# South-Twilight/ParallelWaveGAN

Hardware: AMD Instinct MI355X
Metric: audio samples/sec/GPU (24 kHz PWG, 80-band mel) + RTF at 1/2/4/8 MI355X (higher is better)
Workload: dtype f32 (fp16 hi+lo pair operands, 3 f16 MFMAs per product, fp32 accumulate); 1 GPU; libritts_v1 generator inference, 32 ragged utterances per GPU per step; model=ParallelWaveGANGenerator, hop=300, global_batch=32, frames_per_gpu=24295, parallelism=1 process, 1 GPU (no collective)

## Files before the change

### include/pwg.h

```cpp
#ifndef PWG_H_
#define PWG_H_

#include <stddef.h>

#ifdef __cplusplus
extern "C" {
#endif

#define PWG_ABI_VERSION 2
#if defined(__GNUC__) || defined(__clang__)
#define PWG_API __attribute__((visibility("default")))
#else
#define PWG_API
#endif
#define PWG_MAX_SCALES 8

enum {
  PWG_OK = 0,
  PWG_ERR_INVALID = 1,
  PWG_ERR_ASSERT = 2,
  PWG_ERR_HIP = 3,
  PWG_ERR_UNSUPPORTED = 4,
  PWG_ERR_RANGE = 5,
  PWG_ERR_RERUN = 6
// ... 54 lines not shown
PWG_API long long pwg_plan_workspace_bytes(const PwgPlan* p);

PWG_API int pwg_run(PwgPlan* p, const float* packed, const float* mel, const float* noise,
            const float* mean, const float* scale, float* out, void* workspace, void* stream);

PWG_API int pwg_run_status(PwgPlan* p, const void* workspace, void* stream);

typedef struct PwgGraph PwgGraph;
PWG_API int pwg_graph_create(PwgPlan* p, const float* packed, const float* mel, const float* noise,
                             const float* mean, const float* scale, float* out, void* workspace, void* stream,
                             PwgGraph** out_graph);
PWG_API int pwg_graph_launch(PwgGraph* g, void* stream);
PWG_API void pwg_graph_destroy(PwgGraph* g);

enum {
  PWG_OPT_LAYER_KERNEL = 0,
  PWG_OPT_WAVES_PER_WG = 1,
  PWG_OPT_WG_PER_CU = 2,
  PWG_OPT_FUSE_FIRST_CONV = 3,
  PWG_OPT_PIPELINE = 4,
  PWG_OPT_HALF_BLOCKS = 5,
  PWG_OPT_SYNC = 6,
  PWG_OPT_SYNC_ABORT = 7,
  PWG_OPT_SYNC_TIMEOUT = 8
};
#define PWG_PIPE_MAX_DEFAULT 0LL
PWG_API int pwg_set_option(PwgHandle* h, int option, long long value);
PWG_API int pwg_get_option(const PwgHandle* h, int option, long long* value);

PWG_API int pwg_release_stream(PwgHandle* h, void* stream);
PWG_API int pwg_set_timing(PwgHandle* h, int enable);
PWG_API int pwg_timing_collect(PwgHandle* h, double* ms, long long* launches);
PWG_API int pwg_timing_span(PwgHandle* h, double* span_ms);

#define PWG_RCCL_UNIQUE_ID_BYTES 128
PWG_API int pwg_rccl_unique_id(void* id_out );
PWG_API int pwg_rccl_comm_create(int nranks, const void* id, int rank, int device, void** comm_out);
PWG_API int pwg_rccl_comm_destroy(void* comm);
PWG_API int pwg_broadcast_weights(const PwgHandle* h, void* comm, int root, float* packed, void* stream);

#ifdef __cplusplus
}
#endif
#endif
```

### parallelwavegan_amd/_lib.py

```python

import ctypes
import os
import subprocess
import threading

PKG_DIR = os.path.dirname(os.path.abspath(__file__))
REPO_DIR = os.path.dirname(PKG_DIR)
LIB_DIR = os.path.join(PKG_DIR, "lib")
LIB_PATH = os.environ.get("PWG_LIB_PATH") or os.path.join(LIB_DIR, "libpwg_hip.so")
CSRC = [
    os.path.join(PKG_DIR, "csrc", "pwg_kernels.hip"),
    os.path.join(PKG_DIR, "csrc", "pwg_capi.hip"),
    os.path.join(PKG_DIR, "csrc", "pwg_cnet.hip"),
    os.path.join(PKG_DIR, "csrc", "pwg_split.hip"),
    os.path.join(PKG_DIR, "csrc", "pwg_split16.hip"),
    os.path.join(PKG_DIR, "csrc", "pwg_rccl.hip"),
    os.path.join(PKG_DIR, "csrc", "pwg_mstack.hip"),
    os.path.join(PKG_DIR, "csrc", "pwg_rstack.hip"),
    os.path.join(PKG_DIR, "csrc", "pwg_embed.hip"),
]
HEADERS = [
    os.path.join(REPO_DIR, "include", "pwg.h"),
    os.path.join(REPO_DIR, "include", "pwg_cnet.h"),
    os.path.join(REPO_DIR, "include", "pwg_embed.h"),
# ... 18 lines not shown

EXPORTED_SYMBOLS = (
    "pwg_abi_version",
    "pwg_last_error",
    "pwg_create",
    "pwg_destroy",
    "pwg_receptive_field_size",
    "pwg_upsample_factor",
    "pwg_ref_weight_count",
    "pwg_packed_weight_count",
    "pwg_pack_weights",
    "pwg_plan_create",
    "pwg_plan_destroy",
    "pwg_plan_total_samples",
    "pwg_plan_padded_samples",
    "pwg_plan_workspace_bytes",
    "pwg_run",
    "pwg_run_status",
    "pwg_graph_create",
    "pwg_graph_launch",
    "pwg_graph_destroy",
    "pwg_set_option",
    "pwg_get_option",
    "pwg_set_timing",
    "pwg_release_stream",
    "pwg_timing_collect",
    "pwg_timing_span",
    "pwg_rccl_unique_id",
    "pwg_rccl_comm_create",
    "pwg_rccl_comm_destroy",
    "pwg_broadcast_weights",
    "pwg_cnet_abi_version",
    "pwg_cnet_create",
    "pwg_cnet_destroy",
    "pwg_cnet_packed_weight_count",
    "pwg_cnet_pack_weights",
    "pwg_cnet_plan_create",
    "pwg_cnet_plan_destroy",
    "pwg_cnet_plan_image",
    "pwg_cnet_plan_rows",
    "pwg_cnet_plan_workspace_bytes",
    "pwg_cnet_run",
    "pwg_cnet_run_status",
    "pwg_cnet_plan_schedule",
    "pwg_cnet_set_option",
    "pwg_cnet_set_timing",
    "pwg_cnet_timing_collect",
    "pwg_cnet_timing_span",
    "pwg_cnet_release_stream",
    "pwg_rstack_debug_launches",
    "pwg_rstack_debug_probe",
    "pwg_embed_rows",
)

PWG_OPT_LAYER_KERNEL = 0
PWG_OPT_WAVES_PER_WG = 1
PWG_OPT_WG_PER_CU = 2
PWG_OPT_FUSE_FIRST_CONV = 3
PWG_OPT_PIPELINE = 4
PWG_OPT_HALF_BLOCKS = 5
PWG_OPT_SYNC = 6
PWG_OPT_SYNC_ABORT = 7
PWG_OPT_SYNC_TIMEOUT = 8


class PwgConfig(ctypes.Structure):
    _fields_ = [
        ("in_channels", ctypes.c_int),
        ("out_channels", ctypes.c_int),
        ("kernel_size", ctypes.c_int),
        ("layers", ctypes.c_int),
        ("stacks", ctypes.c_int),
        ("residual_channels", ctypes.c_int),
        ("gate_channels", ctypes.c_int),
        ("skip_channels", ctypes.c_int),
        ("aux_channels", ctypes.c_int),
        ("aux_context_window", ctypes.c_int),
        ("use_causal_conv", ctypes.c_int),
        ("use_conv_in", ctypes.c_int),
        ("num_scales", ctypes.c_int),
        ("upsample_scales", ctypes.c_int * PWG_MAX_SCALES),
        ("interpolate_mode", ctypes.c_int),
    ]


def _needs_build():
# ... 136 lines not shown
        lib.pwg_abi_version.restype = ctypes.c_int
        lib.pwg_last_error.restype = ctypes.c_char_p
        lib.pwg_create.argtypes = [ctypes.POINTER(PwgConfig), ctypes.c_int, ctypes.POINTER(vp)]
        lib.pwg_destroy.argtypes = [vp]
        lib.pwg_destroy.restype = None
        for name in ("pwg_receptive_field_size", "pwg_upsample_factor", "pwg_ref_weight_count",
                     "pwg_packed_weight_count"):
            getattr(lib, name).argtypes = [vp]
            getattr(lib, name).restype = ll
        lib.pwg_pack_weights.argtypes = [vp, vp, vp]
        lib.pwg_plan_create.argtypes = [vp, ctypes.c_int, ctypes.POINTER(ll), ctypes.c_int, ctypes.POINTER(vp)]
        lib.pwg_plan_destroy.argtypes = [vp]
        lib.pwg_plan_destroy.restype = None
        for name in ("pwg_plan_total_samples", "pwg_plan_padded_samples", "pwg_plan_workspace_bytes"):
            getattr(lib, name).argtypes = [vp]
            getattr(lib, name).restype = ll
        lib.pwg_run.argtypes = [vp, vp, vp, vp, vp, vp, vp, vp, vp]
        lib.pwg_run_status.argtypes = [vp, vp, vp]
        lib.pwg_graph_create.argtypes = [vp] * 9 + [ctypes.POINTER(vp)]
        lib.pwg_graph_launch.argtypes = [vp, vp]
        lib.pwg_graph_destroy.argtypes = [vp]
        lib.pwg_graph_destroy.restype = None
        lib.pwg_get_option.argtypes = [vp, ctypes.c_int, ctypes.POINTER(ll)]
        lib.pwg_rccl_unique_id.argtypes = [vp]
        lib.pwg_rccl_comm_create.argtypes = [ctypes.c_int, vp, ctypes.c_int, ctypes.c_int, ctypes.POINTER(vp)]
        lib.pwg_rccl_comm_destroy.argtypes = [vp]
        lib.pwg_broadcast_weights.argtypes = [vp, vp, ctypes.c_int, vp, vp]
        lib.pwg_set_timing.argtypes = [vp, ctypes.c_int]
        lib.pwg_release_stream.argtypes = [vp, vp]
        lib.pwg_set_option.argtypes = [vp, ctypes.c_int, ctypes.c_longlong]
        lib.pwg_timing_collect.argtypes = [vp, ctypes.POINTER(ctypes.c_double), ctypes.POINTER(ll)]
        lib.pwg_timing_span.argtypes = [vp, ctypes.POINTER(ctypes.c_double)]
        lib.pwg_embed_rows.argtypes = [vp, ctypes.c_int, vp, ctypes.c_int, ctypes.c_int, vp, vp, vp, ctypes.c_int, ll,
                                       vp, vp, vp]
        if lib.pwg_abi_version() != 2:
            raise RuntimeError("libpwg_hip ABI version mismatch")
        _lib = lib
        return lib


class RangeError(ArithmeticError):
    """PWG_ERR_RANGE: a value left the fp16 pair range of the split-f16 kernels."""


class RerunError(RuntimeError):
    """PWG_ERR_RERUN: a grid-synchronised or layer-pipelined forward did not complete (the GPU was
# ... 20 lines not shown
```

### parallelwavegan_amd/csrc/pwg_capi.hip

```cpp
#include <hip/hip_runtime.h>

#include <algorithm>
#include <cmath>
#include <cstdio>
#include <cstdlib>
#include <cstring>
#include <map>
#include <mutex>
#include <string>
#include <utility>
#include <vector>

#include "../../include/pwg.h"
#include "pwg_internal.h"

#ifndef PWG_SMALL_SPREAD
#define PWG_SMALL_SPREAD 1
#endif

using namespace pwg;

namespace {

thread_local std::string g_err;
// ... 295 lines not shown

struct PwgHandle {
  PwgConfig cfg;
  int device;
  int R, RS, G, GH, GHPAD, GR, MT, S, SS, M2T, A, KS, KW, O, L, lps, K1, NQ, NQ4;
  long long gap;
  std::vector<int> dil;
  AuxStruct aux;
  size_t off_first_w, off_first_b, off_conv_in, off_conv_in_frag, off_waux;
  size_t off_tab_interior, off_tab_left, off_tab_right, off_tab_small;
  size_t off_layers, layer_stride, lo_wg, lo_bg, lo_w2;
  size_t off_head_w1, off_head_w2, off_head_b2, packed_total;
  int M3T;
  long long ref_total;
  size_t lo_wgp;
  int split_ok = 0;
  size_t lo_split = 0, off_skip0 = 0;
  size_t lo_split16 = 0, off_skip0_16 = 0, off_head16_w1 = 0, off_head16_w2 = 0;
  int layer_kernel = 0, waves_per_wg = 8, wg_per_cu = 1;
  int fuse_first = 1;
  long long pipe_max = PWG_PIPE_MAX_DEFAULT;
  int sync_abort = 0;
  int sync_timeout = 0;
  long long sync_max = -1;
  long long half_max = -1;
  int n_cu = 0;
  int* d_status = nullptr;
  std::string trace_fn;
  unsigned long long* d_trace = nullptr;
  size_t trace_words = 0;
  int timing = 0;
  std::vector<TimingRecord> records;
  std::vector<hipEvent_t> event_pool;
  std::map<hipStream_t, int*> hstatus;
  std::mutex hstatus_mu;
};

struct PwgPlan {
  PwgHandle* h;
  int layout;
  int n_utts;
  std::vector<UttDesc> utts;
  long long n_tiles, n_gap_tiles, Tpad, F_total, T_total;
  size_t ws_x0, ws_x1, ws_skip, ws_c1, ws_d, ws_ctr, ws_flag;
  size_t ws_utts, ws_tile_utt, ws_gap, ws_blocks, ws_total;
  bool pipe_ok = false;
// ... 550 lines not shown
    if (b) h->event_pool.push_back(b);
  };
  if (!a || !b || hipEventRecord(a, s) != hipSuccess) {
    give_back();
    return fail(PWG_ERR_HIP, "timing event");
  }
  const int rc = pwg_run_impl(p, packed, mel, noise, mean, scale, out, workspace, stream);
  if (hipEventRecord(b, s) != hipSuccess) {
    give_back();
    return fail(PWG_ERR_HIP, "timing event");
  }
  h->records.push_back({-1, a, b});
  return rc;
}

static int pwg_run_impl(PwgPlan* p, const float* packed, const float* mel, const float* noise, const float* mean,
                        const float* scale, float* out, void* workspace, void* stream) {
  if (!p || !packed || !mel || !noise || !out || !workspace) return fail(PWG_ERR_INVALID, "null argument");
  if (((uintptr_t)workspace & 255) != 0) return fail(PWG_ERR_INVALID, "workspace must be 256-byte aligned");
  if ((mean == nullptr) != (scale == nullptr)) return fail(PWG_ERR_INVALID, "mean and scale go together");
  if (mean != nullptr && p->layout != PWG_LAYOUT_INFERENCE)
    return fail(PWG_ERR_INVALID, "normalize_before is an inference() option");
  PwgHandle* h = p->h;
  DeviceGuard g(h->device);
  if (!g.ok) return fail(PWG_ERR_HIP, "hipSetDevice failed");
  if (h->n_cu == 0) {
    int n = 0;
    if (hipDeviceGetAttribute(&n, hipDeviceAttributeMultiprocessorCount, h->device) != hipSuccess || n < 1)
      return fail(PWG_ERR_HIP, "cannot query the CU count");
    h->n_cu = n;
  }
  if (h->d_status == nullptr) {
    if (hipMalloc((void**)&h->d_status, 256) != hipSuccess) return fail(PWG_ERR_HIP, "status word allocation");
    if (hipMemset(h->d_status, 0, 256) != hipSuccess) return fail(PWG_ERR_HIP, "status word reset");
  }
  hipStream_t s = (hipStream_t)stream;
  char* ws = (char*)workspace;
  float* x0 = (float*)(ws + p->ws_x0);
  float* x1 = (float*)(ws + p->ws_x1);
  float* skip = (float*)(ws + p->ws_skip);
  float* c1 = (float*)(ws + p->ws_c1);
  float* dproj = (float*)(ws + p->ws_d);
  int* sched_ctr = (int*)(ws + p->ws_ctr);

  auto timed = [&](int bucket, auto&& launch) -> hipError_t {
    if (h->timing != 1) return launch();
// ... 241 lines not shown
      if (fuse_first && l == 0) {
        sa.noise = noise; sa.fw = packed + h->off_first_w; sa.fb = packed + h->off_first_b;
      }
      const int launch_w = split16 ? std::min(8, h->waves_per_wg) : wpw;
      if (split16 && units > 8LL * h->n_cu && units <= 32LL * h->n_cu) wpw = std::min(wpw, 4);
      sa.compute_waves = std::min(wpw, launch_w);
      const bool trace_on = split16 && !h->trace_fn.empty();
      const size_t per_layer_s = (size_t)nwg * launch_w * 8;
      if (trace_on) {
        const size_t need = per_layer_s * 64;
        if (need > h->trace_words) {
          if (h->d_trace) {
            (void)hipStreamSynchronize(s);
            (void)hipFree(h->d_trace);
            h->d_trace = nullptr;
            h->trace_words = 0;
          }
          if (hipMalloc((void**)&h->d_trace, need * sizeof(unsigned long long)) != hipSuccess)
            return fail(PWG_ERR_HIP, "trace buffer");
          h->trace_words = need;
        }
        sa.trace = h->d_trace + per_layer_s * (l % 64);
      }
      e = timed(PWG_KERNEL_RESIDUAL_LAYER, [&] {
        return split16 ? launch_layer_split16(sa, last, la.tap_center, launch_w, nwg, s, half)
                       : launch_layer_split(sa, last, la.tap_center, wpw, nwg, s);
      });
      if (e == hipSuccess && last && trace_on) {
        std::vector<unsigned long long> host(per_layer_s * std::min(h->L, 64));
        e = hipStreamSynchronize(s);
        if (e == hipSuccess) e = hipMemcpy(host.data(), h->d_trace, host.size() * 8, hipMemcpyDeviceToHost);
        FILE* f = e == hipSuccess ? fopen(h->trace_fn.c_str(), "wb") : nullptr;
        if (f) {
          const long long hdr[4] = {std::min(h->L, 64), nwg, launch_w, 8};
          fwrite(hdr, sizeof(hdr), 1, f);
          fwrite(host.data(), 8, host.size(), f);
          fclose(f);
        }
      }
    } else if (h->layer_kernel == 0 && h->aux.nka <= 4) {
      PersistArgs pa2;
      pa2.x_in = xin; pa2.x_out = xout; pa2.skip = skip; pa2.d = la.d;
      pa2.tab = packed + h->off_tab_interior;
      pa2.tab_left = (int)(h->off_tab_left - h->off_tab_interior);
      pa2.tab_right = (int)(h->off_tab_right - h->off_tab_interior);
      pa2.tab_small = (int)(h->off_tab_small - h->off_tab_interior);
      pa2.blocks = d_blocks;
      pa2.wgp = la.wgp; pa2.w2 = la.w2; pa2.bg = la.bg;
// ... 149 lines not shown
      if (value < 1 || value > 64) return fail(PWG_ERR_INVALID, "workgroups per CU must be in [1, 64]");
      h->wg_per_cu = (int)value;
      return PWG_OK;
    case PWG_OPT_PIPELINE:
      if (value < 0) return fail(PWG_ERR_INVALID, "pipeline plan limit must be >= 0");
      h->pipe_max = value;
      return PWG_OK;
    case PWG_OPT_HALF_BLOCKS:
      if (value < 0) return fail(PWG_ERR_INVALID, "half-block limit must be >= 0");
      h->half_max = value;
      return PWG_OK;
    case PWG_OPT_SYNC:
      if (value < 0) return fail(PWG_ERR_INVALID, "grid-synchronised plan limit must be >= 0");
      h->sync_max = value;
      return PWG_OK;
    case PWG_OPT_SYNC_ABORT:
      if (value != 0 && value != 1) return fail(PWG_ERR_INVALID, "sync_abort must be 0 or 1");
      h->sync_abort = (int)value;
      return PWG_OK;
    case PWG_OPT_SYNC_TIMEOUT:
      if (value != 0 && value != 1) return fail(PWG_ERR_INVALID, "sync_timeout must be 0 or 1");
      h->sync_timeout = (int)value;
      return PWG_OK;

    default:
      return fail(PWG_ERR_INVALID, "unknown option");
  }
}

int pwg_get_option(const PwgHandle* h, int option, long long* value) {
  if (!h || !value) return fail(PWG_ERR_INVALID, "null argument");
  switch (option) {
    case PWG_OPT_LAYER_KERNEL: *value = h->layer_kernel; return PWG_OK;
    case PWG_OPT_WAVES_PER_WG: *value = h->waves_per_wg; return PWG_OK;
    case PWG_OPT_FUSE_FIRST_CONV: *value = h->fuse_first; return PWG_OK;
    case PWG_OPT_WG_PER_CU: *value = h->wg_per_cu; return PWG_OK;
    case PWG_OPT_PIPELINE: *value = h->pipe_max; return PWG_OK;
    case PWG_OPT_HALF_BLOCKS: *value = h->half_max >= 0 ? h->half_max : 4LL * h->n_cu; return PWG_OK;
    case PWG_OPT_SYNC: *value = h->sync_max >= 0 ? h->sync_max : 64LL * h->n_cu; return PWG_OK;
    case PWG_OPT_SYNC_ABORT: *value = h->sync_abort; return PWG_OK;
    case PWG_OPT_SYNC_TIMEOUT: *value = h->sync_timeout; return PWG_OK;

    default: return fail(PWG_ERR_INVALID, "unknown option");
  }
}

int pwg_release_stream(PwgHandle* h, void* stream) {
  if (!h) return fail(PWG_ERR_INVALID, "null handle");
  std::lock_guard<std::mutex> lk(h->hstatus_mu);
  auto it = h->hstatus.find((hipStream_t)stream);
  if (it == h->hstatus.end()) return PWG_OK;
  DeviceGuard g(h->device);
  if (stream && hipStreamSynchronize((hipStream_t)stream) != hipSuccess) return fail(PWG_ERR_HIP, "stream synchronize");
  (void)hipHostFree(it->second);
  h->hstatus.erase(it);
  return PWG_OK;
}

int pwg_set_timing(PwgHandle* h, int enable) {
  if (!h) return fail(PWG_ERR_INVALID, "null handle");
  if (enable < 0 || enable > 2) return fail(PWG_ERR_INVALID, "timing mode must be 0, 1 or 2");
  h->timing = enable;
  return PWG_OK;
}

int pwg_timing_collect(PwgHandle* h, double* ms, long long* launches) {
  if (!h || !ms || !launches) return fail(PWG_ERR_INVALID, "null argument");
// ... 60 lines not shown
```

### parallelwavegan_amd/csrc/pwg_internal.h

```cpp
#pragma once
#include <hip/hip_runtime.h>
#include <stdint.h>

namespace pwg {

constexpr int TILE = 128;
constexpr int KC = 16;
constexpr int MAX_SCALES = 8;
constexpr int AUX_J4 = 8;
constexpr int AUX_MAX_NFWG = 16;

struct UttDesc {
  long long seg_base;
  long long first_tile;
  long long T;
  long long frame_base;
  long long frames;
  long long mel_off;
  long long io_off;
};

struct ConvInArgs {
  const float* mel;
  const float* mean;
// ... 180 lines not shown
  UttDesc utts[PLAN_CHUNK];
  int n;
  int u0;
  int gap_tiles;
  int H;
  UttDesc* d_utts;
  int* tile_utt;
  long long* gap_col0;
  BlockDesc* blocks;
  int* zero;
  int n_zero;
  int* prog;
  unsigned* zx[3];
};
hipError_t launch_plan_desc(const PlanDescArgs& a, long long max_blocks, hipStream_t s);

hipError_t launch_conv_in(const ConvInArgs& a, hipStream_t s);
hipError_t launch_aux_proj(const AuxProjArgs& a, int layers, hipStream_t s);
hipError_t launch_first_conv(const FirstConvArgs& a, long long n_tiles, hipStream_t s);
hipError_t launch_layer(const LayerArgs& a, int mt, int m2t, bool last, long long n_tiles, hipStream_t s);
hipError_t launch_first_conv_split(const FirstConvArgs& a, long long n_tiles, hipStream_t s);
hipError_t launch_first_conv_split16(const FirstConvArgs& a, long long n_tiles, hipStream_t s);
hipError_t launch_layer_split16(const SplitArgs& a, bool last, int tap_center, int waves_per_wg, int n_wg,
                                hipStream_t s, bool half = false);
hipError_t launch_layer_split(const SplitArgs& a, bool last, int tap_center, int waves_per_wg, int n_wg,
                              hipStream_t s);
hipError_t launch_pipe_split16(const PipeArgs& p, int tap_center, int n_wg, hipStream_t s);
hipError_t launch_sync_split16(const SyncArgs& p, int tap_center, int n_wg, hipStream_t s);
hipError_t launch_layer_persistent(const PersistArgs& a, int mt, int m2t, bool last, int waves_per_wg, int n_wg,
                                   hipStream_t s);

template <typename V>
__device__ __forceinline__ void stage_lds(V* dst, const V* src, int n, int tid, int nthr) {
  int i = tid;
  for (; i + 7 * nthr < n; i += 8 * nthr) {
    V r[8];
#pragma unroll
    for (int j = 0; j < 8; ++j) r[j] = src[i + j * nthr];
#pragma unroll
    for (int j = 0; j < 8; ++j) dst[i + j * nthr] = r[j];
  }
  for (; i < n; i += nthr) dst[i] = src[i];
}

constexpr int MS_MAX = 4;
struct MsStack {
  const float* wA;
// ... 80 lines not shown
```

### parallelwavegan_amd/csrc/pwg_split16.hip

```cpp
#include "pwg_internal.h"


namespace pwg {

namespace {

typedef float f32x4 __attribute__((ext_vector_type(4)));
typedef _Float16 f16x8 __attribute__((ext_vector_type(8)));
typedef unsigned u32x4 __attribute__((ext_vector_type(4)));

__device__ __forceinline__ f32x4 mma16(u32x4 a, u32x4 b, f32x4 c) {
  return __builtin_amdgcn_mfma_f32_16x16x32_f16(__builtin_bit_cast(f16x8, a), __builtin_bit_cast(f16x8, b), c, 0, 0,
                                                0);
}

__device__ __forceinline__ float gate16(float u, float v) {
  u = fminf(u, 64.f);
  const float e1 = __builtin_amdgcn_exp2f(u);
  const float e2 = __builtin_amdgcn_exp2f(v);
  return (1.f - e1) * __builtin_amdgcn_rcpf((1.f + e1) * (1.f + e2));
}

template <int NOPS>
__device__ __forceinline__ void split8x(const float (&v)[8], u32x4& hi, u32x4& lo) {
// ... 24 lines not shown
  asm volatile(
      "v_fma_mix_f32 %0, %8, %16, %12 op_sel_hi:[1,0,0]\n\t"
      "v_fma_mix_f32 %1, %8, %16, %13 op_sel:[1,0,0] op_sel_hi:[1,0,0]\n\t"
      "v_fma_mix_f32 %2, %9, %16, %14 op_sel_hi:[1,0,0]\n\t"
      "v_fma_mix_f32 %3, %9, %16, %15 op_sel:[1,0,0] op_sel_hi:[1,0,0]\n\t"
      "v_fma_mix_f32 %4, %10, %16, %17 op_sel_hi:[1,0,0]\n\t"
      "v_fma_mix_f32 %5, %10, %16, %18 op_sel:[1,0,0] op_sel_hi:[1,0,0]\n\t"
      "v_fma_mix_f32 %6, %11, %16, %19 op_sel_hi:[1,0,0]\n\t"
      "v_fma_mix_f32 %7, %11, %16, %20 op_sel:[1,0,0] op_sel_hi:[1,0,0]\n\t"
      "v_fma_mix_f32 %0, %21, %16, %0 op_sel_hi:[1,0,0]\n\t"
      "v_fma_mix_f32 %1, %21, %16, %1 op_sel:[1,0,0] op_sel_hi:[1,0,0]\n\t"
      "v_fma_mix_f32 %2, %22, %16, %2 op_sel_hi:[1,0,0]\n\t"
      "v_fma_mix_f32 %3, %22, %16, %3 op_sel:[1,0,0] op_sel_hi:[1,0,0]\n\t"
      "v_fma_mix_f32 %4, %23, %16, %4 op_sel_hi:[1,0,0]\n\t"
      "v_fma_mix_f32 %5, %23, %16, %5 op_sel:[1,0,0] op_sel_hi:[1,0,0]\n\t"
      "v_fma_mix_f32 %6, %24, %16, %6 op_sel_hi:[1,0,0]\n\t"
      "v_fma_mix_f32 %7, %24, %16, %7 op_sel:[1,0,0] op_sel_hi:[1,0,0]\n\t"
      "s_nop 1"
      : "=&v"(o[0]), "=&v"(o[1]), "=&v"(o[2]), "=&v"(o[3]), "=&v"(o[4]), "=&v"(o[5]), "=&v"(o[6]), "=&v"(o[7])
      : "v"(l[0]), "v"(l[1]), "v"(l[2]), "v"(l[3]), "v"(b0[0]), "v"(b0[1]), "v"(b0[2]), "v"(b0[3]), "v"(c),
        "v"(b1[0]), "v"(b1[1]), "v"(b1[2]), "v"(b1[3]), "v"(h[0]), "v"(h[1]), "v"(h[2]), "v"(h[3]));
}

struct Pair16 {
  unsigned hi, lo;
};
__device__ __forceinline__ Pair16 split_pair16(float v0, float v1) {
  typedef _Float16 f16x2 __attribute__((ext_vector_type(2)));
  const _Float16 h0 = (_Float16)v0, h1 = (_Float16)v1;
  const _Float16 l0 = (_Float16)(v0 - (float)h0), l1 = (_Float16)(v1 - (float)h1);
  return {__builtin_bit_cast(unsigned, f16x2{h0, h1}), __builtin_bit_cast(unsigned, f16x2{l0, l1})};
}

}

__device__ __forceinline__ unsigned shifted16(int r, int g, int c) {
  const unsigned s = (unsigned)(r + c);
  return (unsigned)g * 256u + (s >> 4) * 4096u + (s & 15u) * 16u;
}

__device__ __forceinline__ BlockDesc uniform_desc(const BlockDesc& d) {
  BlockDesc u;
  u.col = __builtin_amdgcn_readfirstlane(d.col);
  u.t0 = __builtin_amdgcn_readfirstlane(d.t0);
  u.T = __builtin_amdgcn_readfirstlane(d.T);
  u.frames = __builtin_amdgcn_readfirstlane(d.frames);
// ... 114 lines not shown
#pragma unroll
    for (int m = 0; m < 4; ++m) {
      dv[j][m] = d0[m];
      dv[j][m + 4] = d1[m];
    }
  }
}

template <bool PIPE, int NTN = 2>
__device__ __forceinline__ void s16_load_skip(const SplitArgs& a, const BlockDesc& bd, f32x4 (&sk)[4][2], int g,
                                              int c, int h16 = 0) {
  const Plane16<PIPE> skip(a.skip);
  const long long sb = (long long)((bd.col + h16) >> 4) * 4096;
  const unsigned vo = 16u * (unsigned)(16 * g + c);
#pragma unroll
  for (int nt = 0; nt < NTN; ++nt)
#pragma unroll
    for (int ms = 0; ms < 4; ++ms) {
      if (a.first) sk[ms][nt] = reinterpret_cast<const f32x4*>(a.skip0 + 16 * g)[ms];
      else sk[ms][nt] = __builtin_bit_cast(f32x4, skip.template load<true>(sb + nt * 4096, vo, ms * 1024));
    }
}

template <bool LAST, int TC, bool FIRST, bool PIPE, int NTN = 2, bool AL = false, typename Mid>
__device__ __forceinline__ void s16_block(const SplitArgs& a, const unsigned* smem16, const BlockDesc& bd_v,
                                          const BlockDesc& bdn_v, bool has_next, u32x4 (&b0)[8], u32x4 (&b1)[8],
                                          bool& nonfinite, Mid&& mid, int h16_v = 0, int h16n_v = 0,
                                          bool poison = false) {
  static_assert(NTN == 2 || !LAST, "half blocks: middle layers");
  const BlockDesc bd = uniform_desc(bd_v);
  const int h16 = NTN == 1 ? __builtin_amdgcn_readfirstlane(h16_v) : 0;
  const unsigned* s_wg = smem16;
  const unsigned* s_w2 = s_wg + Split16Smem::WG;
  const unsigned* s_bg = s_w2 + Split16Smem::W2;
  const float* s_bo = reinterpret_cast<const float*>(s_bg + Split16Smem::BG);
  const float* s_hw1 = s_bo + Split16Smem::BO;
  const float* s_fwb = reinterpret_cast<const float*>(smem16 + Split16Smem::dwords(LAST));
  const int lane = threadIdx.x & 63;
  const int g = lane >> 4;
  const int c = lane & 15;
  constexpr int T1 = TC == 1 ? 2 : 1;
  const bool full = bd.t0 + h16 + 16 * NTN <= bd.T;

  unsigned dv[2][8];
  float bw[2][2];
  const bool two_frames = a.H >= 32;
  const int rem0 = bd.t0 - bd.f0 * a.H;
// ... 33 lines not shown
    for (int ks = 0; ks < 2; ++ks) {
#pragma unroll
      for (int mh = 0; mh < 2; ++mh) {
        u32x4 ah[4], al[4];
#pragma unroll
        for (int mm = 0; mm < 4; ++mm) {
          const int m = 4 * mh + mm;
          ah[mm] = wgl[(((tap * 2 + ks) * 8 + m) * 2) * 64];
          al[mm] = wgl[(((tap * 2 + ks) * 8 + m) * 2 + 1) * 64];
        }
#pragma unroll
        for (int mm = 0; mm < 4; ++mm)
#pragma unroll
          for (int nt = 0; nt < NTN; ++nt) {
            f32x4& ac = acc[4 * mh + mm][nt];
            ac = mma16(ah[mm], b[nt * 4 + ks * 2], ac);
            ac = mma16(ah[mm], b[nt * 4 + ks * 2 + 1], ac);
            ac = mma16(al[mm], b[nt * 4 + ks * 2], ac);
          }
        __builtin_amdgcn_sched_barrier(0);
      }
    }
  };

  f32x4 acc[8][2];
#pragma unroll
  for (int m = 0; m < 8; ++m)
#pragma unroll
    for (int nt = 0; nt < NTN; ++nt) acc[m][nt] = f32x4{0.f, 0.f, 0.f, 0.f};
  f32x4 acc2[8][2];
  s16_bload<TC, FIRST, PIPE, NTN, AL>(a, s_fwb, bd, T1, b1, g, c, h16);
  mma_tap(acc, b0, 0);
  s16_load_dv(a, bd, dv, g, c);
  s16_bload<TC, FIRST, PIPE, NTN, AL>(a, s_fwb, bd, TC, b0, g, c, h16);
  mma_tap(acc, b1, T1);
  mma_tap(acc, b0, TC);
  if (!LAST) {
    const f32x4* bo_l = reinterpret_cast<const f32x4*>(s_bo + 16 * g);
#pragma unroll
    for (int nt = 0; nt < NTN; ++nt)
#pragma unroll
      for (int ks = 0; ks < 2; ++ks) {
        float o[8];
        seed8x(b0[nt * 4 + ks * 2], b0[nt * 4 + ks * 2 + 1], bo_l[2 * ks], bo_l[2 * ks + 1], 0.70710677f, o);
#pragma unroll
        for (int j = 0; j < 8; ++j) acc2[4 + 2 * ks + (j >> 2)][nt][j & 3] = o[j];
      }
  }
  mid();

  {
    f32x4 sk[4][2];
    s16_load_skip<PIPE, NTN>(a, bd, sk, g, c, h16);
#pragma unroll
    for (int nt = 0; nt < NTN; ++nt)
#pragma unroll
      for (int ms = 0; ms < 4; ++ms) acc2[ms][nt] = sk[ms][nt];
  }

// ... 18 lines not shown
  }

  u32x4 gh[2][2], gl[2][2];
#pragma unroll
  for (int nt = 0; nt < NTN; ++nt)
#pragma unroll
    for (int ks = 0; ks < 2; ++ks) {
      float gv[8];
#pragma unroll
      for (int j = 0; j < 8; ++j) {
        const int m = 2 * ks + (j >> 2), i = j & 3;
        gv[j] = gate16(acc[m][nt][i], acc[m + 4][nt][i]);
      }
      split8x<0>(gv, gh[nt][ks], gl[nt][ks]);
    }

  if (has_next) {
    const BlockDesc bdn = uniform_desc(bdn_v);
    const int h16n = NTN == 1 ? __builtin_amdgcn_readfirstlane(h16n_v) : 0;
    s16_bload<TC, FIRST, PIPE, NTN, AL>(a, s_fwb, bdn, 0, b0, g, c, h16n);
  }
  constexpr int M2 = LAST ? 4 : 8;
  const u32x4* w2l = reinterpret_cast<const u32x4*>(s_w2) + lane;
#pragma unroll
  for (int ks = 0; ks < 2; ++ks)
#pragma unroll
    for (int mh = 0; mh < M2 / 4; ++mh) {
      u32x4 ah[4], al[4];
#pragma unroll
      for (int mm = 0; mm < 4; ++mm) {
        ah[mm] = w2l[((ks * 8 + 4 * mh + mm) * 2) * 64];
        al[mm] = w2l[((ks * 8 + 4 * mh + mm) * 2 + 1) * 64];
      }
#pragma unroll
      for (int mm = 0; mm < 4; ++mm)
#pragma unroll
        for (int nt = 0; nt < NTN; ++nt) {
          f32x4& ac = acc2[4 * mh + mm][nt];
          ac = mma16(ah[mm], gh[nt][ks], ac);
          ac = mma16(ah[mm], gl[nt][ks], ac);
          ac = mma16(al[mm], gh[nt][ks], ac);
        }
      __builtin_amdgcn_sched_barrier(0);
    }

  if (!LAST) {
    const Plane16<PIPE> skip(a.skip), xo(a.x_out);
    const long long sb = (long long)((bd.col + h16) >> 4) * 4096;
    const unsigned vo = 16u * (unsigned)lane;
#pragma unroll
    for (int nt = 0; nt < NTN; ++nt) {
      const bool live = bd.t0 + h16 + 16 * nt + c < bd.T;
#pragma unroll
      for (int ms = 0; ms < 4; ++ms)
        skip.store(sb + nt * 4096, vo, ms * 1024, __builtin_bit_cast(u32x4, acc2[ms][nt]));
#pragma unroll
      for (int ks = 0; ks < 2; ++ks) {
        float v[8];
#pragma unroll
        for (int j = 0; j < 8; ++j) v[j] = acc2[4 + 2 * ks + (j >> 2)][nt][j & 3];
        u32x4 vh, vl;
        split8x<11>(v, vh, vl);
        if (!full) {
#pragma unroll
          for (int k = 0; k < 4; ++k) {
            vh[k] = live ? vh[k] : 0u;
            vl[k] = live ? vl[k] : 0u;
// ... 49 lines not shown
      }
#pragma unroll
    for (int nt = 0; nt < 2; ++nt) {
      const int t = bd.t0 + 16 * nt + c;
      const bool live = t < bd.T;
      float* out = a.out + (size_t)bd.io_off * a.O + (size_t)t * a.out_stride_t;
      for (int oc = 0; oc < a.O; ++oc) {
        const f32x4* w = reinterpret_cast<const f32x4*>(a.hw2 + ((size_t)oc * 4 + g) * 16);
        float part = 0.f;
#pragma unroll
        for (int m3 = 0; m3 < 4; ++m3) {
          const f32x4 wq = w[m3];
#pragma unroll
          for (int i = 0; i < 4; ++i) part = fmaf(wq[i], fmaxf(acc3[m3][nt][i], 0.f), part);
        }
        part += __shfl_xor(part, 16);
        part += __shfl_xor(part, 32);
        if (g == 0 && live) out[(size_t)oc * a.out_stride_o] = poison ? __builtin_nanf("") : part + a.hb2[oc];
      }
    }
  }
}

template <bool LAST, int TC, bool FIRST, bool AL, int NTN>
__global__ void __launch_bounds__(512, 1) pwg_layer_split16_kernel(const SplitArgs a) {
  constexpr int UB = NTN == 1 ? 1 : 0;
  const int n_units = a.n_blocks << UB;
  extern __shared__ __attribute__((aligned(16))) unsigned smem16[];
  const bool tr = a.trace != nullptr;
  unsigned long long t_start = 0, c_start = 0, t_staged = 0, t_first = 0;
  if (tr) {
    t_start = __builtin_amdgcn_s_memrealtime();
    c_start = __builtin_amdgcn_s_memtime();
  }
  const int lane = threadIdx.x & 63;
  const int nw = a.compute_waves;
  const int xcd = blockIdx.x & 7;
  const int wave = threadIdx.x >> 6;
  const int blk0 = wave < nw ? (int)((long long)n_units * xcd / 8) + (blockIdx.x >> 3) * nw + wave : -1;
  bool poison = false;
  if constexpr (LAST)
    if (a.range_flag != nullptr)
      poison = (__hip_atomic_load(a.range_flag, __ATOMIC_RELAXED, __HIP_MEMORY_SCOPE_AGENT) & PWG_STATUS_REDO) != 0;
  const bool has0 = blk0 >= 0 && blk0 < (int)((long long)n_units * (xcd + 1) / 8);
  BlockDesc bdn;
  int h16n = 0;
  u32x4 b0[8], b1[8];
// ... 47 lines not shown
    return -1;
  };

  int blk = x_first + (blockIdx.x >> 3) * nw + wave;
  int nblk = blk + x_waves;
  if (blk >= x_end) blk = -1;
  if (nblk >= x_end) nblk = -1;
  if (blk < 0) {
    trace_out();
    return;
  }
  const float* s_fwb = reinterpret_cast<const float*>(smem16 + Split16Smem::dwords(LAST));
  if constexpr (FIRST)
    s16_bload<TC, true, false, NTN>(a, s_fwb, uniform_desc(bdn), 0, b0, lane >> 4, lane & 15,
                                    NTN == 1 ? __builtin_amdgcn_readfirstlane(h16n) : 0);
  bool nonfinite = false;
  while (true) {
    const BlockDesc bd = bdn;
    const int h16 = h16n;
    const int pf = nblk >= 0 ? nblk : blk;
    bdn = a.blocks[pf >> UB];
    h16n = NTN == 1 ? 16 * (pf & 1) : 0;
    int ticket = 0;
    s16_block<LAST, TC, FIRST, false, NTN, AL>(a, smem16, bd, bdn, true, b0, b1, nonfinite, [&]() {
      if (nblk >= 0) ticket = ticket_issue();
    }, h16, h16n, poison);
    if (tr && n_done++ == 0) t_first = __builtin_amdgcn_s_memrealtime();
    if (nblk < 0) break;
    blk = nblk;
    nblk = ticket_resolve(ticket);
  }
  if (LAST && nonfinite && a.range_flag) flag_status(a.range_flag, a.sticky, PWG_STATUS_RANGE);
  trace_out();
}

constexpr int PIPE_SPIN_LIMIT = 1 << 20;

template <bool LAST, int TC, bool FIRST>
__device__ __forceinline__ void pipe_layer(const PipeArgs& p, int l, unsigned* smem16) {
  SplitArgs a = p.base;
  a.wg = p.wg0 + (size_t)l * p.wg_stride;
  a.d = p.d0 + (size_t)l * p.d_stride;
  a.x_in = p.x[l % 3];
  a.x_out = p.x[(l + 1) % 3];
  a.dil = p.dil[l];
  a.first = l == 0;
  if (!FIRST) a.noise = nullptr;
// ... 203 lines not shown
    const long long t = t0 + jcol;
    unsigned v = 0u;
    if (t < ud.T) {
      const float z = a.noise[ud.io_off + t];
      float y[2];
#pragma unroll
      for (int e = 0; e < 2; ++e) {
        const int j = 2 * dw + e;
        const int ch = 16 * (2 * ks + (j >> 2)) + 4 * g + (j & 3);
        y[e] = fmaf(a.w[ch], z, a.b[ch]);
      }
      const Pair16 pr = split_pair16(y[0], y[1]);
      v = hl ? pr.lo : pr.hi;
    }
    x[(size_t)col0 * 64 + idx] = v;
  }
}

hipError_t launch_first_conv_split16(const FirstConvArgs& a, long long n_tiles, hipStream_t s) {
  hipLaunchKernelGGL(pwg_first_conv_split16_kernel, dim3((unsigned)n_tiles), dim3(256), 0, s, a);
  return hipGetLastError();
}

hipError_t launch_layer_split16(const SplitArgs& a, bool last, int tap_center, int waves_per_wg, int n_wg,
                                hipStream_t s, bool half) {
  if (waves_per_wg > 8) waves_per_wg = 8;
  if (a.compute_waves < 1 || a.compute_waves > waves_per_wg) return hipErrorInvalidValue;
  if (half && last) return hipErrorInvalidValue;
  const dim3 grid((unsigned)n_wg), block((unsigned)(64 * waves_per_wg));
#define PWG_SPLIT16_LAUNCH(LAST_, TC_, FIRST_, NTN_, AL_)                                               \
  {                                                                                                     \
    const size_t lds = sizeof(unsigned) * (Split16Smem::dwords(LAST_) + (FIRST_ ? 128 : 0));            \
    auto kfn = &pwg_layer_split16_kernel<LAST_, TC_, FIRST_, AL_, NTN_>;                                \
    hipError_t e_ = allow_lds(reinterpret_cast<const void*>(kfn), (int)lds);                           \
    if (e_ != hipSuccess) return e_;                                                                    \
    hipLaunchKernelGGL(kfn, grid, block, lds, s, a);                                                    \
    return hipGetLastError();                                                                           \
  }
  const bool first = a.noise != nullptr;
  if (first && last) return hipErrorInvalidValue;
  const bool al = a.dil % 16 == 0;
#define PWG_SPLIT16_MIDDLE(TC_, NTN_) \
  { if (al) PWG_SPLIT16_LAUNCH(false, TC_, false, NTN_, true) else PWG_SPLIT16_LAUNCH(false, TC_, false, NTN_, false) }
  if (tap_center == 1) {
    if (half) {
      if (first) PWG_SPLIT16_LAUNCH(false, 1, true, 1, false) else PWG_SPLIT16_MIDDLE(1, 1)
    }
    if (first) PWG_SPLIT16_LAUNCH(false, 1, true, 2, false)
    if (last) PWG_SPLIT16_LAUNCH(true, 1, false, 2, false) else PWG_SPLIT16_MIDDLE(1, 2)
  } else if (tap_center == 2) {
    if (half) {
      if (first) PWG_SPLIT16_LAUNCH(false, 2, true, 1, false) else PWG_SPLIT16_MIDDLE(2, 1)
    }
    if (first) PWG_SPLIT16_LAUNCH(false, 2, true, 2, false)
    if (last) PWG_SPLIT16_LAUNCH(true, 2, false, 2, false) else PWG_SPLIT16_MIDDLE(2, 2)
  }
#undef PWG_SPLIT16_MIDDLE
#undef PWG_SPLIT16_LAUNCH
  return hipErrorInvalidValue;
}

hipError_t launch_sync_split16(const SyncArgs& p, int tap_center, int n_wg, hipStream_t s) {
  const size_t lds = sizeof(unsigned) * (Split16Smem::dwords(false) + 128);
  if (p.L < 1 || p.L > PIPE_MAX_LAYERS || p.waves_mid < 1 || p.waves_mid > 8) return hipErrorInvalidValue;
  if (n_wg < 8) return hipErrorInvalidValue;
  auto kfn = tap_center == 1 ? (p.half ? &pwg_sync_split16_kernel<1, 1> : &pwg_sync_split16_kernel<1, 2>)
             : tap_center == 2 ? (p.half ? &pwg_sync_split16_kernel<2, 1> : &pwg_sync_split16_kernel<2, 2>)
                               : nullptr;
  if (kfn == nullptr) return hipErrorInvalidValue;
  const hipError_t e = allow_lds(reinterpret_cast<const void*>(kfn), (int)lds);
  if (e != hipSuccess) return e;
  hipLaunchKernelGGL(kfn, dim3((unsigned)n_wg), dim3(512), lds, s, p);
  return hipGetLastError();
}

hipError_t launch_pipe_split16(const PipeArgs& p, int tap_center, int n_wg, hipStream_t s) {
  const size_t lds = sizeof(unsigned) * (Split16Smem::dwords(true) > Split16Smem::dwords(false) + 128
                                             ? Split16Smem::dwords(true) : Split16Smem::dwords(false) + 128);
  if (n_wg < p.L || n_wg % 8 != 0) return hipErrorInvalidValue;
  auto kfn = tap_center == 1 ? &pwg_pipe_split16_kernel<1> : tap_center == 2 ? &pwg_pipe_split16_kernel<2> : nullptr;
  if (kfn == nullptr) return hipErrorInvalidValue;
// ... 8 lines not shown
```

### parallelwavegan_amd/engine.py

```python

import ctypes
import logging
import os
import operator
from collections import OrderedDict

import numpy as np
import torch

from . import _lib


def _scales(params):
    return list(params.get("upsample_params", {}).get("upsample_scales", [4, 4, 4, 4]))


def make_config(params):
    up = dict(params.get("upsample_params", {"upsample_scales": [4, 4, 4, 4]}))
    if not params.get("upsample_conditional_features", True):
        raise NotImplementedError("upsample_conditional_features=False is not supported")
    net = params.get("upsample_net", "ConvInUpsampleNetwork")
    if net not in ("ConvInUpsampleNetwork", "UpsampleNetwork"):
        raise NotImplementedError(f"upsample_net={net!r} is not supported")
    if up.get("nonlinear_activation") is not None:
# ... 310 lines not shown
    def release_stream(self, stream):
        key = stream.cuda_stream
        self._workspaces.pop(key, None)
        _lib.check(self._lib.pwg_release_stream(self._h, ctypes.c_void_p(key)))

    LAYER_KERNELS = {"persistent": 0, "tiled": 1, "split": 2, "split16": 3}

    def set_option(self, option, value):
        opts = self._OPTS
        if option == "layer_kernel" and isinstance(value, str):
            value = self.LAYER_KERNELS[value]
        if option == "layer_kernel" and int(value) in (2, 3) and not self.split_range_ok:
            raise _lib.RangeError("the loaded weights exceed the fp16 pair range of the split-f16 layer kernels")
        _lib.check(self._lib.pwg_set_option(self._h, opts[option], int(value)))
        if option == "layer_kernel":
            self.layer_kernel = int(value)
        if option == "pipeline":
            self._plans = OrderedDict()

    _OPTS = {"layer_kernel": _lib.PWG_OPT_LAYER_KERNEL, "waves_per_wg": _lib.PWG_OPT_WAVES_PER_WG,
             "wg_per_cu": _lib.PWG_OPT_WG_PER_CU, "fuse_first_conv": _lib.PWG_OPT_FUSE_FIRST_CONV,
             "pipeline": _lib.PWG_OPT_PIPELINE, "half_blocks": _lib.PWG_OPT_HALF_BLOCKS,
             "sync": _lib.PWG_OPT_SYNC, "sync_abort": _lib.PWG_OPT_SYNC_ABORT,
             "sync_timeout": _lib.PWG_OPT_SYNC_TIMEOUT}
    SYNC_FAIL_STREAK = 3
    SYNC_RETRY_RUNS = 256

    def get_option(self, option):
        v = ctypes.c_longlong()
        _lib.check(self._lib.pwg_get_option(self._h, self._OPTS[option], ctypes.byref(v)))
        return int(v.value)

    def set_timing(self, enable):
        self.timing_enabled = bool(enable)
        _lib.check(self._lib.pwg_set_timing(self._h, int(enable)))

    def timing_span(self):
        v = ctypes.c_double()
        _lib.check(self._lib.pwg_timing_span(self._h, ctypes.byref(v)))
        return v.value

    def collect_timing(self):
        ms = (ctypes.c_double * len(_lib.KERNEL_BUCKETS))()
        n = (ctypes.c_longlong * len(_lib.KERNEL_BUCKETS))()
        _lib.check(self._lib.pwg_timing_collect(self._h, ms, n))
        return {k: (ms[i], n[i]) for i, k in enumerate(_lib.KERNEL_BUCKETS)}

    def run(self, plan, mel, noise, out, mean=None, scale=None, stream=None, check=True):
        if stream is None:
            stream = torch.cuda.current_stream(self.device)
        self._sync_tick()
        self._enqueue(plan, mel, noise, out, mean, scale, stream)
        if check:
# ... 191 lines not shown
```

Before: 151.4 million audio samples/s (whole job, all GPUs).

## Prefetch next LDS weight fragment during split-f16 MFMA taps

```diff
diff --git a/include/pwg.h b/include/pwg.h
--- a/include/pwg.h
+++ b/include/pwg.h
@@ -100,11 +100,13 @@
   PWG_OPT_HALF_BLOCKS = 5,
   PWG_OPT_SYNC = 6,
   PWG_OPT_SYNC_ABORT = 7,
-  PWG_OPT_SYNC_TIMEOUT = 8
+  PWG_OPT_SYNC_TIMEOUT = 8,
+  PWG_OPT_FRAGMENT_AHEAD = 9
 };
 #define PWG_PIPE_MAX_DEFAULT 0LL
 PWG_API int pwg_set_option(PwgHandle* h, int option, long long value);
 PWG_API int pwg_get_option(const PwgHandle* h, int option, long long* value);
+PWG_API int pwg_fragment_ahead_launches(const PwgHandle* h, long long* launches);
 
 PWG_API int pwg_release_stream(PwgHandle* h, void* stream);
 PWG_API int pwg_set_timing(PwgHandle* h, int enable);
diff --git a/parallelwavegan_amd/_lib.py b/parallelwavegan_amd/_lib.py
--- a/parallelwavegan_amd/_lib.py
+++ b/parallelwavegan_amd/_lib.py
@@ -64,6 +64,7 @@
     "pwg_graph_destroy",
     "pwg_set_option",
     "pwg_get_option",
+    "pwg_fragment_ahead_launches",
     "pwg_set_timing",
     "pwg_release_stream",
     "pwg_timing_collect",
@@ -104,6 +105,7 @@
 PWG_OPT_SYNC = 6
 PWG_OPT_SYNC_ABORT = 7
 PWG_OPT_SYNC_TIMEOUT = 8
+PWG_OPT_FRAGMENT_AHEAD = 9
 
 
 class PwgConfig(ctypes.Structure):
@@ -286,6 +288,7 @@
         lib.pwg_graph_destroy.argtypes = [vp]
         lib.pwg_graph_destroy.restype = None
         lib.pwg_get_option.argtypes = [vp, ctypes.c_int, ctypes.POINTER(ll)]
+        lib.pwg_fragment_ahead_launches.argtypes = [vp, ctypes.POINTER(ll)]
         lib.pwg_rccl_unique_id.argtypes = [vp]
         lib.pwg_rccl_comm_create.argtypes = [ctypes.c_int, vp, ctypes.c_int, ctypes.c_int, ctypes.POINTER(vp)]
         lib.pwg_rccl_comm_destroy.argtypes = [vp]
diff --git a/parallelwavegan_amd/csrc/pwg_capi.hip b/parallelwavegan_amd/csrc/pwg_capi.hip
--- a/parallelwavegan_amd/csrc/pwg_capi.hip
+++ b/parallelwavegan_amd/csrc/pwg_capi.hip
@@ -341,6 +341,8 @@
   long long pipe_max = PWG_PIPE_MAX_DEFAULT;
   int sync_abort = 0;
   int sync_timeout = 0;
+  int frag_ahead = 1;
+  long long fa_launches = 0;
   long long sync_max = -1;
   long long half_max = -1;
   int n_cu = 0;
@@ -937,6 +939,7 @@
   if (mean != nullptr && p->layout != PWG_LAYOUT_INFERENCE)
     return fail(PWG_ERR_INVALID, "normalize_before is an inference() option");
   PwgHandle* h = p->h;
+  h->fa_launches = 0;
   DeviceGuard g(h->device);
   if (!g.ok) return fail(PWG_ERR_HIP, "hipSetDevice failed");
   if (h->n_cu == 0) {
@@ -1224,8 +1227,11 @@
         }
         sa.trace = h->d_trace + per_layer_s * (l % 64);
       }
+      const bool frag_ahead =
+          split16 && h->frag_ahead && split16_has_fragment_ahead(last, sa.noise != nullptr, half);
+      if (frag_ahead) ++h->fa_launches;
       e = timed(PWG_KERNEL_RESIDUAL_LAYER, [&] {
-        return split16 ? launch_layer_split16(sa, last, la.tap_center, launch_w, nwg, s, half)
+        return split16 ? launch_layer_split16(sa, last, la.tap_center, launch_w, nwg, s, half, frag_ahead)
                        : launch_layer_split(sa, last, la.tap_center, wpw, nwg, s);
       });
       if (e == hipSuccess && last && trace_on) {
@@ -1421,6 +1427,10 @@
       if (value != 0 && value != 1) return fail(PWG_ERR_INVALID, "sync_timeout must be 0 or 1");
       h->sync_timeout = (int)value;
       return PWG_OK;
+    case PWG_OPT_FRAGMENT_AHEAD:
+      if (value != 0 && value != 1) return fail(PWG_ERR_INVALID, "fragment_ahead must be 0 or 1");
+      h->frag_ahead = (int)value;
+      return PWG_OK;
 
     default:
       return fail(PWG_ERR_INVALID, "unknown option");
@@ -1439,9 +1449,16 @@
     case PWG_OPT_SYNC: *value = h->sync_max >= 0 ? h->sync_max : 64LL * h->n_cu; return PWG_OK;
     case PWG_OPT_SYNC_ABORT: *value = h->sync_abort; return PWG_OK;
     case PWG_OPT_SYNC_TIMEOUT: *value = h->sync_timeout; return PWG_OK;
+    case PWG_OPT_FRAGMENT_AHEAD: *value = h->frag_ahead; return PWG_OK;
 
     default: return fail(PWG_ERR_INVALID, "unknown option");
   }
+}
+
+int pwg_fragment_ahead_launches(const PwgHandle* h, long long* launches) {
+  if (!h || !launches) return fail(PWG_ERR_INVALID, "null argument");
+  *launches = h->fa_launches;
+  return PWG_OK;
 }
 
 int pwg_release_stream(PwgHandle* h, void* stream) {
diff --git a/parallelwavegan_amd/csrc/pwg_internal.h b/parallelwavegan_amd/csrc/pwg_internal.h
--- a/parallelwavegan_amd/csrc/pwg_internal.h
+++ b/parallelwavegan_amd/csrc/pwg_internal.h
@@ -226,7 +226,8 @@
 hipError_t launch_first_conv_split(const FirstConvArgs& a, long long n_tiles, hipStream_t s);
 hipError_t launch_first_conv_split16(const FirstConvArgs& a, long long n_tiles, hipStream_t s);
 hipError_t launch_layer_split16(const SplitArgs& a, bool last, int tap_center, int waves_per_wg, int n_wg,
-                                hipStream_t s, bool half = false);
+                                hipStream_t s, bool half = false, bool frag_ahead = false);
+bool split16_has_fragment_ahead(bool last, bool first, bool half);
 hipError_t launch_layer_split(const SplitArgs& a, bool last, int tap_center, int waves_per_wg, int n_wg,
                               hipStream_t s);
 hipError_t launch_pipe_split16(const PipeArgs& p, int tap_center, int n_wg, hipStream_t s);
diff --git a/parallelwavegan_amd/csrc/pwg_split16.hip b/parallelwavegan_amd/csrc/pwg_split16.hip
--- a/parallelwavegan_amd/csrc/pwg_split16.hip
+++ b/parallelwavegan_amd/csrc/pwg_split16.hip
@@ -70,6 +70,35 @@
         "v"(b1[0]), "v"(b1[1]), "v"(b1[2]), "v"(b1[3]), "v"(h[0]), "v"(h[1]), "v"(h[2]), "v"(h[3]));
 }
 
+template <int OFF>
+__device__ __forceinline__ void fa_read(u32x4& h, u32x4& l, unsigned addr) {
+  static_assert(OFF >= 0 && OFF + 1024 < 65536, "ds_read offset field");
+  asm volatile(
+      "s_nop 6\n\t"
+      "ds_read_b128 %0, %2 offset:%3\n\t"
+      "ds_read_b128 %1, %2 offset:%4"
+      : "=&v"(h), "=&v"(l)
+      : "v"(addr), "i"(OFF), "i"(OFF + 1024));
+}
+template <int N>
+__device__ __forceinline__ void fa_wait(u32x4& h, u32x4& l) {
+  asm volatile("s_waitcnt lgkmcnt(%2)" : "+v"(h), "+v"(l) : "i"(N));
+}
+__device__ __forceinline__ unsigned lds_addr(const void* p) {
+  return (unsigned)(size_t)(__attribute__((address_space(3))) const void*)p;
+}
+template <int I>
+struct IC {
+  static constexpr int value = I;
+};
+template <int I, int N, typename F>
+__device__ __forceinline__ void fa_for(F&& f) {
+  if constexpr (I < N) {
+    f(IC<I>{});
+    fa_for<I + 1, N>(f);
+  }
+}
+
 struct Pair16 {
   unsigned hi, lo;
 };
@@ -230,7 +259,7 @@
     }
 }
 
-template <bool LAST, int TC, bool FIRST, bool PIPE, int NTN = 2, bool AL = false, typename Mid>
+template <bool LAST, int TC, bool FIRST, bool PIPE, int NTN = 2, bool AL = false, bool FA = false, typename Mid>
 __device__ __forceinline__ void s16_block(const SplitArgs& a, const unsigned* smem16, const BlockDesc& bd_v,
                                           const BlockDesc& bdn_v, bool has_next, u32x4 (&b0)[8], u32x4 (&b1)[8],
                                           bool& nonfinite, Mid&& mid, int h16_v = 0, int h16n_v = 0,
@@ -310,6 +339,26 @@
       }
     }
   };
+  constexpr int FA_IMG = 2 * 8 * 2 * 64 * 16;
+  const unsigned fa_base = FA ? lds_addr(smem16) + 16u * (unsigned)lane : 0u;
+  u32x4 fh[2], fl[2];
+  auto mma_tap_fa = [&](f32x4 (&acc)[8][2], const u32x4 (&b)[8], int tap, int nxt) {
+    const unsigned here = fa_base + (unsigned)(tap * FA_IMG), there = fa_base + (unsigned)(nxt * FA_IMG);
+    fa_for<0, 16>([&](auto sc) {
+      constexpr int s = decltype(sc)::value, ks = s >> 3, m = s & 7, cur = s & 1;
+      if constexpr (s < 15) fa_read<(s + 1) * 2048>(fh[cur ^ 1], fl[cur ^ 1], here);
+      else fa_read<0>(fh[cur ^ 1], fl[cur ^ 1], there);
+      fa_wait<2>(fh[cur], fl[cur]);
+#pragma unroll
+      for (int nt = 0; nt < NTN; ++nt) {
+        f32x4& ac = acc[m][nt];
+        ac = mma16(fh[cur], b[nt * 4 + ks * 2], ac);
+        ac = mma16(fh[cur], b[nt * 4 + ks * 2 + 1], ac);
+        ac = mma16(fl[cur], b[nt * 4 + ks * 2], ac);
+      }
+      __builtin_amdgcn_sched_barrier(0);
+    });
+  };
 
   f32x4 acc[8][2];
 #pragma unroll
@@ -317,12 +366,19 @@
 #pragma unroll
     for (int nt = 0; nt < NTN; ++nt) acc[m][nt] = f32x4{0.f, 0.f, 0.f, 0.f};
   f32x4 acc2[8][2];
+  if constexpr (FA) fa_read<0>(fh[0], fl[0], fa_base);
   s16_bload<TC, FIRST, PIPE, NTN, AL>(a, s_fwb, bd, T1, b1, g, c, h16);
-  mma_tap(acc, b0, 0);
+  if constexpr (FA) mma_tap_fa(acc, b0, 0, T1);
+  else mma_tap(acc, b0, 0);
   s16_load_dv(a, bd, dv, g, c);
   s16_bload<TC, FIRST, PIPE, NTN, AL>(a, s_fwb, bd, TC, b0, g, c, h16);
-  mma_tap(acc, b1, T1);
-  mma_tap(acc, b0, TC);
+  if constexpr (FA) {
+    mma_tap_fa(acc, b1, T1, TC);
+    mma_tap_fa(acc, b0, TC, 3);
+  } else {
+    mma_tap(acc, b1, T1);
+    mma_tap(acc, b0, TC);
+  }
   if (!LAST) {
     const f32x4* bo_l = reinterpret_cast<const f32x4*>(s_bo + 16 * g);
 #pragma unroll
@@ -387,6 +443,27 @@
   }
   constexpr int M2 = LAST ? 4 : 8;
   const u32x4* w2l = reinterpret_cast<const u32x4*>(s_w2) + lane;
+  if constexpr (FA) {
+    const unsigned here = fa_base + 3u * FA_IMG;
+    fa_for<0, 2 * M2>([&](auto sc) {
+      constexpr int s = decltype(sc)::value, ks = s / M2, m = s % M2, cur = s & 1;
+      constexpr int sn = s + 1, fn = (sn / M2) * 8 + sn % M2;
+      if constexpr (sn < 2 * M2) {
+        fa_read<fn * 2048>(fh[cur ^ 1], fl[cur ^ 1], here);
+        fa_wait<2>(fh[cur], fl[cur]);
+      } else {
+        fa_wait<0>(fh[cur], fl[cur]);
+      }
+#pragma unroll
+      for (int nt = 0; nt < NTN; ++nt) {
+        f32x4& ac = acc2[m][nt];
+        ac = mma16(fh[cur], gh[nt][ks], ac);
+        ac = mma16(fh[cur], gl[nt][ks], ac);
+        ac = mma16(fl[cur], gh[nt][ks], ac);
+      }
+      __builtin_amdgcn_sched_barrier(0);
+    });
+  } else {
 #pragma unroll
   for (int ks = 0; ks < 2; ++ks)
 #pragma unroll
@@ -408,6 +485,7 @@
         }
       __builtin_amdgcn_sched_barrier(0);
     }
+  }
 
   if (!LAST) {
     const Plane16<PIPE> skip(a.skip), xo(a.x_out);
@@ -503,7 +581,7 @@
   }
 }
 
-template <bool LAST, int TC, bool FIRST, bool AL, int NTN>
+template <bool LAST, int TC, bool FIRST, bool AL, bool FA, int NTN>
 __global__ void __launch_bounds__(512, 1) pwg_layer_split16_kernel(const SplitArgs a) {
   constexpr int UB = NTN == 1 ? 1 : 0;
   const int n_units = a.n_blocks << UB;
@@ -597,7 +675,7 @@
     bdn = a.blocks[pf >> UB];
     h16n = NTN == 1 ? 16 * (pf & 1) : 0;
     int ticket = 0;
-    s16_block<LAST, TC, FIRST, false, NTN, AL>(a, smem16, bd, bdn, true, b0, b1, nonfinite, [&]() {
+    s16_block<LAST, TC, FIRST, false, NTN, AL, FA>(a, smem16, bd, bdn, true, b0, b1, nonfinite, [&]() {
       if (nblk >= 0) ticket = ticket_issue();
     }, h16, h16n, poison);
     if (tr && n_done++ == 0) t_first = __builtin_amdgcn_s_memrealtime();
@@ -847,23 +925,36 @@
   return hipGetLastError();
 }
 
+constexpr bool FA_MIDDLE = true, FA_LAST = true, FA_FIRST_HALF = true, FA_FIRST_WHOLE = true;
+
+bool split16_has_fragment_ahead(bool last, bool first, bool half) {
+  return last ? FA_LAST : first ? (half ? FA_FIRST_HALF : FA_FIRST_WHOLE) : FA_MIDDLE;
+}
+
 hipError_t launch_layer_split16(const SplitArgs& a, bool last, int tap_center, int waves_per_wg, int n_wg,
-                                hipStream_t s, bool half) {
+                                hipStream_t s, bool half, bool frag_ahead) {
   if (waves_per_wg > 8) waves_per_wg = 8;
   if (a.compute_waves < 1 || a.compute_waves > waves_per_wg) return hipErrorInvalidValue;
   if (half && last) return hipErrorInvalidValue;
   const dim3 grid((unsigned)n_wg), block((unsigned)(64 * waves_per_wg));
-#define PWG_SPLIT16_LAUNCH(LAST_, TC_, FIRST_, NTN_, AL_)                                               \
+#define PWG_SPLIT16_LAUNCH_FA(LAST_, TC_, FIRST_, NTN_, AL_, FA_)                                       \
   {                                                                                                     \
     const size_t lds = sizeof(unsigned) * (Split16Smem::dwords(LAST_) + (FIRST_ ? 128 : 0));            \
-    auto kfn = &pwg_layer_split16_kernel<LAST_, TC_, FIRST_, AL_, NTN_>;                                \
+    auto kfn = &pwg_layer_split16_kernel<LAST_, TC_, FIRST_, AL_, FA_, NTN_>;                           \
     hipError_t e_ = allow_lds(reinterpret_cast<const void*>(kfn), (int)lds);                           \
     if (e_ != hipSuccess) return e_;                                                                    \
     hipLaunchKernelGGL(kfn, grid, block, lds, s, a);                                                    \
     return hipGetLastError();                                                                           \
   }
+#define PWG_SPLIT16_LAUNCH(LAST_, TC_, FIRST_, NTN_, AL_)                                               \
+  {                                                                                                     \
+    if constexpr (LAST_ ? FA_LAST : FIRST_ ? (NTN_ == 1 ? FA_FIRST_HALF : FA_FIRST_WHOLE) : FA_MIDDLE) \
+      if (frag_ahead) PWG_SPLIT16_LAUNCH_FA(LAST_, TC_, FIRST_, NTN_, AL_, true)                        \
+    PWG_SPLIT16_LAUNCH_FA(LAST_, TC_, FIRST_, NTN_, AL_, false)                                         \
+  }
   const bool first = a.noise != nullptr;
   if (first && last) return hipErrorInvalidValue;
+  if (frag_ahead && !split16_has_fragment_ahead(last, first, half)) return hipErrorInvalidValue;
   const bool al = a.dil % 16 == 0;
 #define PWG_SPLIT16_MIDDLE(TC_, NTN_) \
   { if (al) PWG_SPLIT16_LAUNCH(false, TC_, false, NTN_, true) else PWG_SPLIT16_LAUNCH(false, TC_, false, NTN_, false) }
@@ -882,6 +973,7 @@
   }
 #undef PWG_SPLIT16_MIDDLE
 #undef PWG_SPLIT16_LAUNCH
+#undef PWG_SPLIT16_LAUNCH_FA
   return hipErrorInvalidValue;
 }
 
diff --git a/parallelwavegan_amd/engine.py b/parallelwavegan_amd/engine.py
--- a/parallelwavegan_amd/engine.py
+++ b/parallelwavegan_amd/engine.py
@@ -356,13 +356,18 @@
              "wg_per_cu": _lib.PWG_OPT_WG_PER_CU, "fuse_first_conv": _lib.PWG_OPT_FUSE_FIRST_CONV,
              "pipeline": _lib.PWG_OPT_PIPELINE, "half_blocks": _lib.PWG_OPT_HALF_BLOCKS,
              "sync": _lib.PWG_OPT_SYNC, "sync_abort": _lib.PWG_OPT_SYNC_ABORT,
-             "sync_timeout": _lib.PWG_OPT_SYNC_TIMEOUT}
+             "sync_timeout": _lib.PWG_OPT_SYNC_TIMEOUT, "fragment_ahead": _lib.PWG_OPT_FRAGMENT_AHEAD}
     SYNC_FAIL_STREAK = 3
     SYNC_RETRY_RUNS = 256
 
     def get_option(self, option):
         v = ctypes.c_longlong()
         _lib.check(self._lib.pwg_get_option(self._h, self._OPTS[option], ctypes.byref(v)))
+        return int(v.value)
+
+    def fragment_ahead_launches(self):
+        v = ctypes.c_longlong()
+        _lib.check(self._lib.pwg_fragment_ahead_launches(self._h, ctypes.byref(v)))
         return int(v.value)
 
     def set_timing(self, enable):
```

Result: faster. 154.4 million audio samples/s (whole job, all GPUs), median of 6 (+2.0%).
